# ai-dynamo/dynamo

Measured on AMD Instinct MI355X. Metric: output tok/s (node), Llama-3-70B serving, ISL8192/OSL1024, conc 16/GPU, higher is better.
Workload: dtype bf16; 1 GPU; model=llama-3-70b, global_batch=16, seq_len=8192, osl=1024, parallelism=agg1, kv_cache_dtype=auto

## Files before the change

### dynamo_amd/csrc/attention_decode.hip

```cpp
#include "attention_decode_impl.h"
#include <torch/extension.h>
#include <ATen/hip/HIPContext.h>

using namespace decode_attn;

int64_t paged_decode_num_chunks(int64_t max_ctx) {
  const int chunk = decode_chunk_tokens((int)max_ctx);
  return std::max<int64_t>(1, (max_ctx + chunk - 1) / chunk);
}

int64_t decode_chunk_tokens_py(int64_t max_ctx) {
  return decode_chunk_tokens((int)max_ctx);
}

void paged_attention_decode(torch::Tensor out, torch::Tensor q,
                            torch::Tensor kcache, torch::Tensor vcache,
                            torch::Tensor page_table, torch::Tensor ctx_lens,
                            torch::Tensor partial, torch::Tensor ml,
                            double scale, int64_t chunk_tokens,
                            bool v_transposed,
                            c10::optional<torch::Tensor> chunk_cnt) {
  TORCH_CHECK(q.is_cuda() && q.dtype() == torch::kBFloat16);
  TORCH_CHECK(page_table.dtype() == torch::kInt32 && ctx_lens.dtype() == torch::kInt32);
  const bool fp8 = kcache.dtype() == torch::kFloat8_e4m3fn;
  TORCH_CHECK(fp8 || kcache.dtype() == torch::kBFloat16,
              "kv cache must be bf16 or float8_e4m3fn");
  const int B = q.size(0);
  const int Hq = q.size(1);
  const int hd = q.size(2);
  const int Hkv = kcache.size(1);
  const int ps = kcache.size(2);
  const int G = Hq / Hkv;
  const int max_pages = page_table.size(1);
  const int C = ml.size(2);
  TORCH_CHECK(hd == 128, "only head_dim=128 supported natively");
  TORCH_CHECK((ps & (ps - 1)) == 0, "page_size must be a power of 2");
  int log2_ps = 0; while ((1 << log2_ps) < ps) log2_ps++;
  if (B == 0) return;
  const int chunk = (int)chunk_tokens;
  TORCH_CHECK(chunk >= 128 && chunk % 128 == 0, "bad chunk_tokens ", chunk);
  auto stream = at::cuda::getCurrentHIPStream();
  dim3 grid(B, Hkv, C);

  if (v_transposed) {
    TORCH_CHECK(vcache.size(2) == hd && vcache.size(3) == ps,
                "v_transposed expects vcache [P, Hkv, hd, ps]");
    TORCH_CHECK(ps % 32 == 0 && hd == 128 && G >= 2 && G <= 16,
                "v_transposed decode needs page_size%32==0, head_dim==128, "
                "2<=G<=16 (got G=", G, ")");
    const int lds = mfma_swapped_lds_bytes(G, hd, 72);
    static const bool use_fused_merge = [] {
      const char* e = getenv("DYNAMO_FUSED_MERGE");
      return e != nullptr && e[0] == '1';
    }();
    int32_t* cnt = nullptr;
    if (use_fused_merge && C > 1 && chunk_cnt.has_value() &&
        chunk_cnt->numel() >= (int64_t)B * Hkv)
      cnt = chunk_cnt->data_ptr<int32_t>();
    auto launch_vt = [&](auto* kern) {
      if (lds > 65536)
        (void)hipFuncSetAttribute(reinterpret_cast<const void*>(kern),
                                  hipFuncAttributeMaxDynamicSharedMemorySize,
                                  lds);
      kern<<<grid, kBlock, lds, stream>>>(
          partial.data_ptr<float>(), ml.data_ptr<float>(),
          (short*)out.data_ptr(), (const short*)q.data_ptr(),
          (const short*)kcache.data_ptr(), (const short*)vcache.data_ptr(),
          page_table.data_ptr<int32_t>(), ctx_lens.data_ptr<int32_t>(),
          (float)scale, chunk, G, B, Hkv, C, max_pages, log2_ps, hd, cnt);
    };
    static const int vt3v = [] {
      const char* e = getenv("DYNAMO_VT3_VARIANT");
      return e ? atoi(e) : 0;
    }();
    if (fp8)
      launch_vt(&paged_decode_mfma_swapped<1, 1, 0, 1, 72, 0, 4>);
    else if (vt3v == 1)
      launch_vt(&paged_decode_mfma_swapped<1, 1, 0, 0, 72, 0, 3, 0, 2>);
    else if (vt3v == 2)
      launch_vt(&paged_decode_mfma_swapped<1, 1, 0, 0, 72, 0, 2>);
    else if (vt3v == 5 && ps == 64)
      launch_vt(&paged_decode_mfma_swapped<1, 1, 0, 0, 72, 0, 5>);
    else
      launch_vt(&paged_decode_mfma_swapped<1, 1, 0, 0, 72, 0, 4>);
    HIP_CHECK_KERNEL();
    if (C > 1 && cnt == nullptr) {
      dim3 grid2(B, Hq);
      paged_decode_phase2<<<grid2, 128, 0, stream>>>(
          (short*)out.data_ptr(), partial.data_ptr<float>(),
          ml.data_ptr<float>(), ctx_lens.data_ptr<int32_t>(), chunk, Hq, C,
          hd);
      HIP_CHECK_KERNEL();
    }
    return;
  }

#define LAUNCH_G(GG, DP, HS, DEPTH)                                           \
  paged_decode_phase1<GG, DP, HS, DEPTH>                                      \
      <<<grid, kBlock, phase1_lds_bytes(GG, HS, hd), stream>>>(               \
      partial.data_ptr<float>(), ml.data_ptr<float>(), (short*)out.data_ptr(),\
      (const short*)q.data_ptr(), (const short*)kcache.data_ptr(),            \
      (const short*)vcache.data_ptr(), page_table.data_ptr<int32_t>(),        \
      ctx_lens.data_ptr<int32_t>(), (float)scale, chunk, B, Hkv, C,            \
      max_pages, log2_ps, hd)
  static const bool use_mfma = [] {
    const char* e = getenv("DYNAMO_DECODE_MFMA");
    return e == nullptr || e[0] != '0';
  }();
  static const bool use_swapped = [] {
    const char* e = getenv("DYNAMO_DECODE_SWAPPED");
    return e == nullptr || e[0] != '0';
  }();
#define LAUNCH_MFMA(GG)                                                       \
  do {                                                                        \
    if (use_swapped) {                                                        \
      if (mfma_swapped_lds_bytes(GG, hd, 72) > 65536)                             \
        (void)hipFuncSetAttribute(                                            \
            reinterpret_cast<const void*>(                                    \
                &paged_decode_mfma_swapped<1, 1, 0, 0, 72, 1>),                         \
            hipFuncAttributeMaxDynamicSharedMemorySize,                       \
            mfma_swapped_lds_bytes(GG, hd, 72));                                  \
      paged_decode_mfma_swapped<1, 1, 0, 0, 72, 1>                                      \
          <<<grid, kBlock, mfma_swapped_lds_bytes(GG, hd, 72), stream>>>(         \
          partial.data_ptr<float>(), ml.data_ptr<float>(),                    \
          (short*)out.data_ptr(), (const short*)q.data_ptr(),                 \
          (const short*)kcache.data_ptr(),                                    \
          (const short*)vcache.data_ptr(), page_table.data_ptr<int32_t>(),    \
          ctx_lens.data_ptr<int32_t>(), (float)scale, chunk, GG, B, Hkv, C,    \
          max_pages, log2_ps, hd, nullptr);                                   \
      break;                                                                  \
    }                                                                         \
    if (mfma_lds_bytes(GG, hd) > 65536)                                       \
      (void)hipFuncSetAttribute(                                              \
          reinterpret_cast<const void*>(&paged_decode_mfma<1, 1>),            \
          hipFuncAttributeMaxDynamicSharedMemorySize,                         \
          mfma_lds_bytes(GG, hd));                                            \
    paged_decode_mfma<1, 1><<<grid, kBlock, mfma_lds_bytes(GG, hd), stream>>>(\
      partial.data_ptr<float>(), ml.data_ptr<float>(), (short*)out.data_ptr(),\
      (const short*)q.data_ptr(), (const short*)kcache.data_ptr(),            \
      (const short*)vcache.data_ptr(), page_table.data_ptr<int32_t>(),        \
      ctx_lens.data_ptr<int32_t>(), (float)scale, chunk, GG, B, Hkv, C,        \
      max_pages, log2_ps, hd);                                                \
  } while (0)
  const bool mfma_ok = use_mfma && ps % 32 == 0 && hd == 128;
  if (fp8) {
    TORCH_CHECK(ps % 32 == 0 && hd == 128 && G <= 16,
                "fp8 KV cache needs page_size%32==0, head_dim==128, G<=16");
    if (mfma_swapped_lds_bytes(G, hd, 72) > 65536)
      (void)hipFuncSetAttribute(
          reinterpret_cast<const void*>(&paged_decode_mfma_swapped<1, 1, 0, 1, 72, 1>),
          hipFuncAttributeMaxDynamicSharedMemorySize,
          mfma_swapped_lds_bytes(G, hd, 72));
    paged_decode_mfma_swapped<1, 1, 0, 1, 72, 1>
        <<<grid, kBlock, mfma_swapped_lds_bytes(G, hd, 72), stream>>>(
        partial.data_ptr<float>(), ml.data_ptr<float>(),
        (short*)out.data_ptr(), (const short*)q.data_ptr(),
        (const short*)kcache.data_ptr(), (const short*)vcache.data_ptr(),
        page_table.data_ptr<int32_t>(), ctx_lens.data_ptr<int32_t>(),
        (float)scale, chunk, G, B, Hkv, C, max_pages, log2_ps, hd, nullptr);
// ... 43 lines not shown
```

### dynamo_amd/csrc/attention_decode_impl.h

```cpp
#pragma once
#include "common.h"
#include <cstdlib>

namespace decode_attn {

constexpr int kBlock = 256;

inline int decode_chunk_tokens(int max_ctx) {
#ifndef __HIP_DEVICE_COMPILE__
  if (const char* e = getenv("DYNAMO_DECODE_CHUNK")) {
    const int v = atoi(e);
    if (v >= 128 && v % 128 == 0) return v;
  }
#endif
  if (max_ctx >= 8192) return 2048;
  if (max_ctx >= 2048) return 1024;
  return 512;
}
#ifndef DECODE_KCHUNK
#define DECODE_KCHUNK 512
#endif
constexpr int kChunk = DECODE_KCHUNK;
constexpr float kNegInf = -1e30f;

// ... 389 lines not shown
      *(short*)((char*)p_lds + row * 64 + (((16 + lr) * 2) ^ x)) = f32_to_bf16(pB[r]);
    }
    __builtin_amdgcn_wave_barrier();
    asm volatile("s_waitcnt lgkmcnt(0)" ::: "memory");
    __builtin_amdgcn_sched_barrier(0);

    if (active) {
    short8 pa_s;
    {
      const int row = lr;
      const int x = (row & 3) << 4;
      pa_s = *reinterpret_cast<const short8*>(
          (char*)p_lds + row * 64 + ((lg * 16) ^ x));
    }
    bf16x8_t pa = *reinterpret_cast<bf16x8_t*>(&pa_s);
    if constexpr (PRIO) __builtin_amdgcn_s_setprio(1);
#pragma unroll
    for (int db = 0; db < 8; db++) {
      short8 vb_s = *reinterpret_cast<const short8*>(
          (const char*)v_lds + (db * 16 + lr) * 80 + lg * 16);
      bf16x8_t vbf = *reinterpret_cast<bf16x8_t*>(&vb_s);
      acc[db] = __builtin_amdgcn_mfma_f32_16x16x32_bf16(pa, vbf, acc[db],
                                                        0, 0, 0);
    }
    if constexpr (PRIO) __builtin_amdgcn_s_setprio(0);
    }
    __builtin_amdgcn_wave_barrier();
  }

  __syncthreads();
  float* my = merge + wid * G * (hd + 2);
#pragma unroll
  for (int r = 0; r < 4; r++) {
    const int row = lg * 4 + r;
    if (row < G) {
#pragma unroll
      for (int db = 0; db < 8; db++)
        my[row * (hd + 2) + db * 16 + lr] = acc[db][r];
      if (lr == 0) {
        my[row * (hd + 2) + hd] = m[r];
        my[row * (hd + 2) + hd + 1] = l[r];
      }
    }
  }
  __syncthreads();

  for (int i = threadIdx.x; i < G * hd; i += kBlock) {
    const int g = i / hd;
    const int d = i % hd;
    float mw[4], lw[4];
    float mstar = kNegInf;
#pragma unroll
    for (int w = 0; w < 4; w++) {
      mw[w] = merge[w * G * (hd + 2) + g * (hd + 2) + hd];
      lw[w] = merge[w * G * (hd + 2) + g * (hd + 2) + hd + 1];
      mstar = fmaxf(mstar, mw[w]);
    }
    float lsum = 0.f, asum = 0.f;
#pragma unroll
    for (int w = 0; w < 4; w++) {
      const float corr = (lw[w] > 0.f) ? __expf(mw[w] - mstar) : 0.f;
      lsum += lw[w] * corr;
      asum += merge[w * G * (hd + 2) + g * (hd + 2) + d] * corr;
    }
    const int qh = h * G + g;
    if (C == 1) {
      out[((int64_t)b * Hq + qh) * hd + d] =
          f32_to_bf16(lsum > 0.f ? asum / lsum : 0.f);
    } else {
      partial[(((int64_t)b * Hq + qh) * C + c) * hd + d] = asum;
      if (d == 0) {
        float* mlp = ml + (((int64_t)b * Hq + qh) * C + c) * 2;
        mlp[0] = mstar; mlp[1] = lsum;
      }
    }
  }
}

inline int mfma_lds_bytes(int G, int hd) {
  return 4 * G * (hd + 2) * 4 + G * hd * 2 + 4 * 5120 * 2 + 4 * 512 * 2;
}

template <int DEFER = 1, int PRIO = 1, int KPF = 0, int FP8 = 0,
          int VS = 80, int XK2 = 0, int VT = 0, int LG2 = 0, int MINW = 1>
__global__ __launch_bounds__(kBlock, MINW) void paged_decode_mfma_swapped(
    float* __restrict__ partial, float* __restrict__ ml,
    short* __restrict__ out, const short* __restrict__ q,
    const short* __restrict__ kcache, const short* __restrict__ vcache,
    const int32_t* __restrict__ page_table, const int32_t* __restrict__ ctx_lens,
    float scale, int chunk, int G, int B, int Hkv, int C, int max_pages,
    int log2_ps, int hd, int32_t* __restrict__ chunk_cnt) {
  typedef __attribute__((ext_vector_type(8))) __bf16 bf16x8_t;
  typedef __attribute__((ext_vector_type(2))) unsigned int uint2_t;
  const int kSlab = chunk / 4;
  const int b = blockIdx.x;
  const int h = blockIdx.y;
  const int c = blockIdx.z;
  const int Hq = Hkv * G;
  const int ctx = ctx_lens[b];
  const int chunk_start = c * chunk;
  const int lane = threadIdx.x & 63;
  const int wid = threadIdx.x >> 6;
  const int lr = lane & 15;
  const int lg = lane >> 4;
  const int ps = 1 << log2_ps;

  extern __shared__ float lds[];
  float* merge = lds;
  short* q_lds_s = reinterpret_cast<short*>(merge + 4 * G * (hd + 2));
  short* v_lds = q_lds_s + G * hd + wid * (hd * VS / 2);

  auto fused_merge = [&]() {
    __threadfence();
    __shared__ int lastflag;
    if (threadIdx.x == 0) {
      const int prev = atomicAdd(&chunk_cnt[b * Hkv + h], 1);
      lastflag = (prev == (int)gridDim.z - 1) ? 1 : 0;
    }
    __syncthreads();
    if (!lastflag) return;
    __threadfence();
    if (threadIdx.x == 0) chunk_cnt[b * Hkv + h] = 0;
    const int nc = min(C, (ctx + chunk - 1) / chunk);
    for (int i = threadIdx.x; i < G * hd; i += kBlock) {
      const int g = i / hd;
      const int d = i % hd;
      const int qh = h * G + g;
      const float* mlp = ml + (((int64_t)b * Hq + qh) * C) * 2;
      float mstar = kNegInf;
      for (int cc = 0; cc < nc; cc++) mstar = fmaxf(mstar, mlp[2 * cc]);
      float asum = 0.f, lsum2 = 0.f;
      for (int cc = 0; cc < nc; cc++) {
        const float lc = mlp[2 * cc + 1];
        if (lc <= 0.f) continue;
        const float corr = __expf(mlp[2 * cc] - mstar);
        asum += partial[(((int64_t)b * Hq + qh) * C + cc) * hd + d] * corr;
        lsum2 += lc * corr;
      }
      out[((int64_t)b * Hq + qh) * hd + d] =
          f32_to_bf16(lsum2 > 0.f ? asum / lsum2 : 0.f);
    }
  };

  if (chunk_start >= ctx) {
    if (C > 1) {
      for (int i = threadIdx.x; i < G; i += kBlock) {
        const int qh = h * G + i;
        float* mlp = ml + (((int64_t)b * Hq + qh) * C + c) * 2;
        mlp[0] = kNegInf; mlp[1] = 0.f;
      }
      if (chunk_cnt != nullptr) fused_merge();
    }
    return;
  }

  for (int i = threadIdx.x; i < G * hd; i += kBlock) {
    const int g = i / hd;
    q_lds_s[i] = q[((int64_t)b * Hq + h * G + g) * hd + i % hd];
  }
  __syncthreads();

  bf16x8_t q_frag[4];
#pragma unroll
  for (int kc = 0; kc < 4; kc++) {
    short8 v{};
    if (lr < G)
      v = *reinterpret_cast<const short8*>(q_lds_s + lr * hd + kc * 32 + lg * 8);
    q_frag[kc] = *reinterpret_cast<bf16x8_t*>(&v);
  }

  float m_run = kNegInf, l_run = 0.f;
  f32x4 acc[8];
#pragma unroll
  for (int d = 0; d < 8; d++) acc[d] = f32x4{0.f, 0.f, 0.f, 0.f};

  const int slab_start = chunk_start + wid * kSlab;
  const int slab_end = min(slab_start + kSlab, ctx);
  const int32_t* pt = page_table + (int64_t)b * max_pages;

  typedef __attribute__((ext_vector_type(4))) short short4v;
  auto ld8 = [&](const short* base, int64_t elem_off) -> short8 {
    if constexpr (FP8) {
      const unsigned char* b =
          reinterpret_cast<const unsigned char*>(base) + elem_off;
      uchar8 raw = *reinterpret_cast<const uchar8*>(b);
      bf16x8 cv = fp8x8_to_bf16x8(raw);
      return *reinterpret_cast<short8*>(&cv);
    } else {
      return *reinterpret_cast<const short8*>(base + elem_off);
    }
  };
  auto load_k = [&](int t0_, short8 (&kf)[8]) {
    if (t0_ >= slab_end) return;
    const int64_t pb = (((int64_t)pt[t0_ >> log2_ps] * Hkv + h) * ps) * hd;
    const int tA = t0_ + lr, tB = t0_ + 16 + lr;
    const int64_t oA = pb + (int64_t)(tA & (ps - 1)) * hd;
    const int64_t oB = pb + (int64_t)(tB & (ps - 1)) * hd;
    const bool vA = tA < slab_end, vB = tB < slab_end;
#pragma unroll
    for (int kc = 0; kc < 4; kc++) {
      kf[kc] = vA ? ld8(kcache, oA + kc * 32 + lg * 8) : short8{};
      kf[4 + kc] = vB ? ld8(kcache, oB + kc * 32 + lg * 8) : short8{};
    }
  };
  auto load_v = [&](int t0_, short8 (&vf)[8]) {
    if (t0_ >= slab_end) return;
    const int64_t pb = (((int64_t)pt[t0_ >> log2_ps] * Hkv + h) * ps) * hd;
#pragma unroll
    for (int u = 0; u < 2; u++) {
      const int unit = lane + u * 64;
      const int d8 = unit & 15;
      const int tg = unit >> 4;
#pragma unroll
      for (int j = 0; j < 4; j++) {
        const int t = t0_ + tg * 4 + j;
        vf[u * 4 + j] = (t < slab_end)
            ? ld8(vcache, pb + (int64_t)(t & (ps - 1)) * hd + d8 * 8)
            : short8{};
      }
    }
  };
  auto load_vt = [&](int t0_, short8 (&vf)[8]) {
    const int64_t pb = (((int64_t)pt[t0_ >> log2_ps] * Hkv + h) * ps) * hd;
    const int tin = t0_ & (ps - 1);
#pragma unroll
    for (int da = 0; da < 8; da++) {
      const int vrow = da * 16 + lr;
      vf[da] = ld8(vcache, pb + (int64_t)vrow * ps + tin + lg * 8);
    }
    const int rem = slab_end - t0_;
    if (rem < 32) {
#pragma unroll
      for (int da = 0; da < 8; da++)
#pragma unroll
        for (int j = 0; j < 8; j++)
          if (lg * 8 + j >= rem) vf[da][j] = 0;
    }
  };
  auto store_v = [&](const short8 (&vf)[8]) {
#pragma unroll
    for (int u = 0; u < 2; u++) {
      const int unit = lane + u * 64;
      const int d8 = unit & 15;
      const int tg = unit >> 4;
#pragma unroll
      for (int i = 0; i < 8; i++) {
        const int d = d8 * 8 + i;
        short4v pk = {vf[u * 4 + 0][i], vf[u * 4 + 1][i],
                      vf[u * 4 + 2][i], vf[u * 4 + 3][i]};
        const int toff = XK2 ? ((tg * 8) ^ (((d >> 4) & 1) << 5)) : (tg * 8);
        *reinterpret_cast<short4v*>((char*)v_lds + d * VS + toff) = pk;
      }
    }
  };

  short8 kfr[2][8], vfr[2][8];
  if constexpr (KPF) {
    load_k(slab_start, kfr[0]);
    load_v(slab_start, vfr[0]);
  }

  const float scale2 = scale * 1.44269504f;
  auto tile_vt = [&](int t0, const short8 (&kf)[8], const short8 (&vf)[8]) {
    f32x4 sA{0.f, 0.f, 0.f, 0.f}, sB{0.f, 0.f, 0.f, 0.f};
    if constexpr (PRIO) __builtin_amdgcn_s_setprio(1);
#pragma unroll
    for (int kc = 0; kc < 4; kc++) {
      short8 ka = kf[kc];
      sA = __builtin_amdgcn_mfma_f32_16x16x32_bf16(
          *reinterpret_cast<bf16x8_t*>(&ka), q_frag[kc], sA, 0, 0, 0);
    }
    if (t0 + 16 < slab_end) {
// ... 613 lines not shown
```

### dynamo_amd/csrc/bindings.cpp

```cpp
#include <torch/extension.h>
#include <pybind11/pybind11.h>

namespace py = pybind11;

void rmsnorm(torch::Tensor out, torch::Tensor input, torch::Tensor weight,
             double eps, bool allow_fast);
void fused_add_rmsnorm(torch::Tensor input, torch::Tensor residual,
                       torch::Tensor weight, double eps, bool allow_fast);
void rope_append_qkv(torch::Tensor q_out, torch::Tensor kcache,
                     torch::Tensor vcache, torch::Tensor qkv,
                     c10::optional<torch::Tensor> bias,
                     torch::Tensor positions, torch::Tensor slot_mapping,
                     torch::Tensor cos_sin_cache, bool v_transposed,
                     bool allow_fast);
void rope_inplace(torch::Tensor q, torch::Tensor k, torch::Tensor positions,
                  torch::Tensor cos_sin_cache, int64_t num_q_heads,
                  int64_t num_k_heads, int64_t head_dim);
void silu_mul(torch::Tensor out, torch::Tensor gate_up);
void gelu(torch::Tensor out, torch::Tensor input);
void kv_cache_append(torch::Tensor kcache, torch::Tensor vcache, torch::Tensor k,
                     torch::Tensor v, torch::Tensor slot_mapping,
                     bool v_transposed);
void gather_pages(torch::Tensor staging, torch::Tensor cache, torch::Tensor page_ids);
void scatter_pages(torch::Tensor staging, torch::Tensor cache, torch::Tensor page_ids);
void copy_pages(torch::Tensor dst_cache, torch::Tensor src_cache, torch::Tensor pairs);
int64_t paged_decode_num_chunks(int64_t max_ctx);
int64_t decode_chunk_tokens_py(int64_t max_ctx);
void paged_attention_decode(torch::Tensor out, torch::Tensor q, torch::Tensor kcache,
                            torch::Tensor vcache, torch::Tensor page_table,
                            torch::Tensor ctx_lens, torch::Tensor partial,
                            torch::Tensor ml, double scale,
                            int64_t chunk_tokens, bool v_transposed,
                            c10::optional<torch::Tensor> chunk_cnt);
void attention_prefill_paged(torch::Tensor out, torch::Tensor q,
                             torch::Tensor kcache, torch::Tensor vcache,
                             torch::Tensor page_table, torch::Tensor tile_seq,
                             torch::Tensor tile_q0, torch::Tensor seq_q_start,
                             torch::Tensor seq_q_len, torch::Tensor seq_ctx_len,
                             double scale, bool v_transposed);
void greedy_sample(torch::Tensor out, torch::Tensor logits, bool allow_fast);
void topkp_sample(torch::Tensor out, torch::Tensor logits,
                  torch::Tensor inv_temp, torch::Tensor top_k,
                  torch::Tensor top_p, int64_t seed,
                  c10::optional<torch::Tensor> row_seeds);
void gumbel_sample(torch::Tensor out, torch::Tensor logits, torch::Tensor inv_temp,
                   int64_t seed, c10::optional<torch::Tensor> row_seeds,
                   bool allow_fast);
void moe_grouped_gemm(torch::Tensor y, torch::Tensor x, torch::Tensor w,
                      torch::Tensor tiles);
void moe_grouped_gemm_seg(torch::Tensor y, torch::Tensor x, torch::Tensor w,
                          torch::Tensor seg_start, int64_t max_tokens);
void topk_gating(torch::Tensor topw, torch::Tensor topi, torch::Tensor logits);
torch::Tensor ipc_alloc(int64_t nbytes, int64_t device);
py::bytes ipc_export(torch::Tensor t);
torch::Tensor ipc_open(py::bytes handle_bytes, int64_t nbytes, int64_t device);
void enable_peer_access(int64_t device, int64_t peer);
torch::Tensor mfma_probe(torch::Tensor A, torch::Tensor B);
torch::Tensor tr16_probe();
torch::Tensor vstage_probe();
torch::Tensor pv_probe(int64_t hot);

PYBIND11_MODULE(TORCH_EXTENSION_NAME, m) {
  m.doc() = "dynamo_amd native MI355X (gfx950) kernels";
  m.def("rmsnorm", &rmsnorm, py::arg("out"), py::arg("input"),
        py::arg("weight"), py::arg("eps"), py::arg("allow_fast") = true);
  m.def("fused_add_rmsnorm", &fused_add_rmsnorm, py::arg("input"),
        py::arg("residual"), py::arg("weight"), py::arg("eps"),
        py::arg("allow_fast") = true);
  m.def("rope_inplace", &rope_inplace);
  m.def("rope_append_qkv", &rope_append_qkv,
        py::arg("q_out"), py::arg("kcache"), py::arg("vcache"),
        py::arg("qkv"), py::arg("bias"), py::arg("positions"),
        py::arg("slot_mapping"), py::arg("cos_sin"),
        py::arg("v_transposed") = false, py::arg("allow_fast") = true);
  m.def("silu_mul", &silu_mul);
  m.def("gelu", &gelu);
  m.def("kv_cache_append", &kv_cache_append, py::arg("kcache"),
        py::arg("vcache"), py::arg("k"), py::arg("v"),
        py::arg("slot_mapping"), py::arg("v_transposed") = false);
  m.def("gather_pages", &gather_pages);
  m.def("scatter_pages", &scatter_pages);
  m.def("copy_pages", &copy_pages);
  m.def("paged_decode_num_chunks", &paged_decode_num_chunks);
  m.def("decode_chunk_tokens", &decode_chunk_tokens_py);
  m.def("paged_attention_decode", &paged_attention_decode,
        py::arg("out"), py::arg("q"), py::arg("kcache"), py::arg("vcache"),
        py::arg("page_table"), py::arg("ctx_lens"), py::arg("partial"),
        py::arg("ml"), py::arg("scale"), py::arg("chunk_tokens"),
        py::arg("v_transposed") = false,
        py::arg("chunk_cnt") = py::none());
  m.def("attention_prefill_paged", &attention_prefill_paged,
        py::arg("out"), py::arg("q"), py::arg("kcache"), py::arg("vcache"),
        py::arg("page_table"), py::arg("tile_seq"), py::arg("tile_q0"),
        py::arg("seq_q_start"), py::arg("seq_q_len"), py::arg("seq_ctx_len"),
        py::arg("scale"), py::arg("v_transposed") = false);
  m.def("greedy_sample", &greedy_sample, py::arg("out"), py::arg("logits"),
        py::arg("allow_fast") = true);
  m.def("gumbel_sample", &gumbel_sample, py::arg("out"), py::arg("logits"),
        py::arg("inv_temp"), py::arg("seed"),
        py::arg("row_seeds") = py::none(), py::arg("allow_fast") = true);
  m.def("topkp_sample", &topkp_sample, py::arg("out"), py::arg("logits"),
        py::arg("inv_temp"), py::arg("top_k"), py::arg("top_p"),
        py::arg("seed"), py::arg("row_seeds") = py::none());
  m.def("moe_grouped_gemm", &moe_grouped_gemm);
  m.def("moe_grouped_gemm_seg", &moe_grouped_gemm_seg);
  m.def("topk_gating", &topk_gating);
  m.def("ipc_alloc", &ipc_alloc);
  m.def("ipc_export", &ipc_export);
  m.def("ipc_open", &ipc_open);
  m.def("enable_peer_access", &enable_peer_access);
  m.def("mfma_probe", &mfma_probe);
  m.def("tr16_probe", &tr16_probe);
  m.def("vstage_probe", &vstage_probe);
  m.def("pv_probe", &pv_probe);
}
```

### dynamo_amd/envs.py

```python
from __future__ import annotations

import os

ENV_VARS = {
    "DYN_DISCOVERY_BACKEND": "discovery backend spec: memory | file:/path",
    "DYN_NAMESPACE": "default namespace for components",
    "DYN_LOG": "log level (INFO, DEBUG, ...)",
    "DYN_LOGGING_JSONL": "1 = structured JSONL logs",
    "DYN_REQUEST_TRACE_FILE": "JSONL request-trace sink path",
    "DYN_HTTP_PORT": "frontend HTTP port",
    "DYN_ROUTER_MODE": "kv | round_robin | random | least_loaded | p2c",
    "DYN_ROUTER_TEMPERATURE": "softmax temperature for kv routing",
    "DYN_KV_BLOCK_SIZE": "KV page size in tokens",
    "DYN_KV_GPU_MEM_FRACTION": "fraction of free HBM for the KV pool",
    "DYN_HOST_CACHE_PAGES": "KVBM G2 pinned-host tier size (pages)",
    "DYN_TUNABLEOP": "0 disables the pre-tuned hipBLASLt table",
    "DYN_WORKER_TYPE": "aggregated | prefill | decode",
    "DYN_BYPASS_TOKEN_THRESHOLD":
        "conditional disagg: net-new prefill tokens below this bypass the "
        "prefill pool (reference conditional_disagg.rs:15; default 2048)",
    "DYNAMO_DECODE_CHUNK": "decode attention context-chunk tokens override",
    "DYNAMO_DECODE_MFMA": "0 = force the VALU decode path (token-major only)",
    "DYNAMO_DECODE_SWAPPED": "0 = A-operand MFMA decode (token-major only)",
    "DYNAMO_VT3_VARIANT":
        "d-major decode variant select: 0=VT4 (default), 1=VT3, 2=VT2, "
        "5=VT5 (recorded-negative V-LDS variant)",
    "DYNAMO_FUSED_MERGE":
        "1 = fused decode chunk merge (recorded-negative; threadfence cost)",
    "DYNAMO_MOE_BMM": "0 = grouped-kernel MoE decode instead of padded bmm",
    "DYNAMO_MOE_MFMA": "0 = VALU grouped MoE GEMM",
    "DYNAMO_MOE_GRAPHS": "0 = exclude MoE layers from hipGraph capture",
    "DYNAMO_ROCTX": "1 = roctx range annotations for rocprofv3 traces",
}


def get(name: str, default=None, cast=str):
    v = os.environ.get(name)
    if v is None:
        return default
    try:
        if cast is bool:
            return v not in ("0", "false", "False", "")
        return cast(v)
    except (TypeError, ValueError):
        return default


def discovery(default="memory"):
    return get("DYN_DISCOVERY_BACKEND", default)


def namespace(default="dynamo"):
    return get("DYN_NAMESPACE", default)
```

### dynamo_amd/models/layers.py

```python
from __future__ import annotations

from dataclasses import dataclass, field
from typing import List, Optional

import torch
import torch.nn.functional as F

from dynamo_amd import ops


@dataclass
class AttnMetadata:
    slot_mapping: torch.Tensor
    positions: torch.Tensor
    num_decode: int = 0
    decode_page_table: Optional[torch.Tensor] = None
    decode_ctx_lens: Optional[torch.Tensor] = None
    decode_scratch: Optional["ops.DecodeScratch"] = None
    num_prefill_tokens: int = 0
    prefill_page_table: Optional[torch.Tensor] = None
    seq_q_start: Optional[torch.Tensor] = None
    seq_q_len: Optional[torch.Tensor] = None
    seq_ctx_len: Optional[torch.Tensor] = None
    prefill_tiles: Optional[tuple] = None
    logits_rows: Optional[torch.Tensor] = None
    embeds_rows: Optional[torch.Tensor] = None
    inputs_embeds: Optional[torch.Tensor] = None
    v_transposed: bool = False


def linear(x: torch.Tensor, w: torch.Tensor) -> torch.Tensor:
    return F.linear(x, w)


def linear_lora(x: torch.Tensor, w: torch.Tensor, lora, key: str) -> torch.Tensor:
    y = F.linear(x, w)
    if lora is not None and key in lora:
        A, B, scale = lora[key]
        y = y + F.linear(F.linear(x, A), B) * scale
    return y


class TPContext:

    def __init__(self, tp_size: int = 1, tp_rank: int = 0, group=None):
        self.size = tp_size
        self.rank = tp_rank
        self.group = group

    def all_reduce(self, x: torch.Tensor) -> torch.Tensor:
        if self.size > 1:
            torch.distributed.all_reduce(x, group=self.group)
        return x


_DEFAULT_TP = TPContext()


def _alloc(shape, device, dtype):
    from dynamo_amd.gms import current_allocator
    pool = current_allocator()
    if pool is not None:
        return pool.allocate(shape, dtype), pool.needs_init
    return torch.empty(shape, device=device, dtype=dtype), True


def init_weight(shape, device, dtype, std=0.02, generator=None):
    from dynamo_amd.gms import current_allocator
    pooled = current_allocator() is not None
    w, needs = _alloc(shape, device, dtype)
    if needs:
        with torch.no_grad():
            if pooled:
                tmp = torch.empty(shape, device=device, dtype=dtype)
                tmp.normal_(0.0, std, generator=generator)
                w.copy_(tmp)
            else:
                w.normal_(0.0, std, generator=generator)
    return w


def init_const(shape, device, dtype, val=1.0):
    w, needs = _alloc(shape, device, dtype)
    if needs:
        with torch.no_grad():
            w.fill_(val)
    return w


def init_sharded(shape, device, dtype, tp: "TPContext", dim: int, std=0.02):
    if tp.size == 1:
        return init_weight(shape, device, dtype, std)
    n = shape[dim] // tp.size
    shard_shape = list(shape)
    shard_shape[dim] = n
    shard, needs = _alloc(tuple(shard_shape), device, dtype)
    if needs:
        full = torch.empty(shape, device=device, dtype=dtype)
        with torch.no_grad():
            full.normal_(0.0, std)
        shard.copy_(full.narrow(dim, tp.rank * n, n))
        del full
    return shard


class Attention(torch.nn.Module):

    def __init__(self, cfg, layer_idx: int, tp: TPContext, device, dtype):
        super().__init__()
        self.layer_idx = layer_idx
        self.tp = tp
        self.hq = cfg.num_q_heads // tp.size
        self.hkv = max(1, cfg.num_kv_heads // tp.size)
        self.hd = cfg.head_dim
        self.scale = self.hd ** -0.5
        D = cfg.hidden_size
        qkv_rows = (self.hq + 2 * self.hkv) * self.hd
        kv_idx = (tp.rank if tp.size <= cfg.num_kv_heads
                  else (tp.rank * cfg.num_kv_heads) // tp.size)
# ... 84 lines not shown
```

### dynamo_amd/ops/__init__.py

```python
from __future__ import annotations

import torch

from . import torch_ref
from .torch_ref import make_cos_sin_cache

_hip_mod = None
_hip_err: Exception | None = None


def hip():
    global _hip_mod, _hip_err
    if _hip_mod is None:
        try:
            from dynamo_amd import _hip as m
            _hip_mod = m
        except Exception as e:
            _hip_err = e
            raise RuntimeError(
                "dynamo_amd._hip native extension is not available on a GPU "
                "device path. Build it with `python setup.py build_ext "
                f"--inplace` (PYTORCH_ROCM_ARCH=gfx950). Original error: {e}"
            ) from e
    return _hip_mod


def hip_available() -> bool:
    try:
        hip()
        return True
    except RuntimeError:
        return False


def rmsnorm(x: torch.Tensor, weight: torch.Tensor, eps: float,
            allow_fast: bool = True) -> torch.Tensor:
    if x.is_cuda:
        out = torch.empty_like(x)
        hip().rmsnorm(out, x.contiguous(), weight, eps, allow_fast)
        return out
    return torch_ref.rmsnorm(x, weight, eps)


def fused_add_rmsnorm(x, residual, weight, eps, allow_fast=True):
    if x.is_cuda:
        hip().fused_add_rmsnorm(x, residual, weight, eps, allow_fast)
        return x
    return torch_ref.fused_add_rmsnorm(x, residual, weight, eps)


def rope_inplace(q, k, positions, cos_sin, num_q_heads, num_k_heads, head_dim):
    if q.is_cuda:
        hip().rope_inplace(q, k, positions, cos_sin, num_q_heads, num_k_heads,
                           head_dim)
        return q, k
    return torch_ref.rope(q, k, positions, cos_sin, num_q_heads, num_k_heads,
                          head_dim)


def silu_mul(gate_up: torch.Tensor) -> torch.Tensor:
    if gate_up.is_cuda:
        d = gate_up.shape[-1] // 2
        out = torch.empty(gate_up.shape[:-1] + (d,), dtype=gate_up.dtype,
                          device=gate_up.device)
        hip().silu_mul(out, gate_up.contiguous())
        return out
    return torch_ref.silu_mul(gate_up)


def gelu(x: torch.Tensor) -> torch.Tensor:
    if x.is_cuda:
        out = torch.empty_like(x)
        hip().gelu(out, x.contiguous())
        return out
    return torch_ref.gelu(x)


def kv_cache_append(kcache, vcache, k, v, slot_mapping,
                    v_transposed=False):
    if kcache.is_cuda:
        hip().kv_cache_append(kcache, vcache, k.contiguous(), v.contiguous(),
                              slot_mapping, v_transposed)
    else:
        torch_ref.kv_cache_append(kcache, vcache, k, v, slot_mapping,
                                  v_transposed)


def rope_append_qkv(qkv, bias, positions, slot_mapping, cos_sin,
                    kcache, vcache, num_q_heads, num_kv_heads, head_dim,
                    v_transposed=False, allow_fast=True):
    T = qkv.shape[0]
    if qkv.is_cuda:
        q_out = torch.empty(T, num_q_heads * head_dim, dtype=qkv.dtype,
                            device=qkv.device)
        hip().rope_append_qkv(q_out, kcache, vcache, qkv, bias, positions,
                              slot_mapping, cos_sin, v_transposed, allow_fast)
        return q_out
    if bias is not None:
        qkv = qkv + bias
    q, k, v = qkv.split([num_q_heads * head_dim, num_kv_heads * head_dim,
                         num_kv_heads * head_dim], dim=-1)
    q = q.contiguous()
    k = k.contiguous()
    q, k = torch_ref.rope(q, k, positions, cos_sin, num_q_heads,
                          num_kv_heads, head_dim)
    torch_ref.kv_cache_append(kcache, vcache, k.view(T, num_kv_heads, head_dim),
                              v.view(T, num_kv_heads, head_dim), slot_mapping,
                              v_transposed)
    return q


class DecodeScratch:

    def __init__(self, max_batch: int, num_q_heads: int, head_dim: int,
                 max_ctx: int, device):
        self.chunks = int(hip().paged_decode_num_chunks(max_ctx))
        self.chunk_tokens = int(hip().decode_chunk_tokens(max_ctx))
        self.partial = torch.empty(max_batch, num_q_heads, self.chunks, head_dim,
                                   dtype=torch.float32, device=device)
        self.ml = torch.empty(max_batch, num_q_heads, self.chunks, 2,
                              dtype=torch.float32, device=device)
        self.chunk_cnt = torch.zeros(max_batch * 128, dtype=torch.int32,
                                     device=device)

    def view(self, batch: int):
        return self.partial[:batch], self.ml[:batch]


def paged_attention_decode(q, kcache, vcache, page_table, ctx_lens, scale,
                           scratch: "DecodeScratch | None" = None, out=None,
                           v_transposed=False):
    if q.is_cuda:
        if out is None:
            out = torch.empty_like(q)
        assert scratch is not None, "GPU decode needs a DecodeScratch"
        partial, ml = scratch.view(q.shape[0])
        hip().paged_attention_decode(out, q, kcache, vcache, page_table,
                                     ctx_lens, partial, ml, scale,
                                     scratch.chunk_tokens, v_transposed,
                                     scratch.chunk_cnt)
        return out
    r = torch_ref.paged_attention_decode(q, kcache, vcache, page_table,
                                         ctx_lens, scale,
                                         v_transposed=v_transposed)
    if out is not None:
        out.copy_(r)
        return out
    return r


def prefill_tile_rows(num_q_heads: int, num_kv_heads: int) -> int:
    if num_q_heads % num_kv_heads == 0:
        g = num_q_heads // num_kv_heads
        if g in (2, 4, 8):
            return (8 // g) * 32
    return 64


def build_prefill_tiles(seq_q_lens, device, rows: int = 64):
    tile_seq, tile_q0 = [], []
    for s, ql in enumerate(seq_q_lens):
        for q0 in range(0, int(ql), rows):
            tile_seq.append(s)
            tile_q0.append(q0)
    return (torch.tensor(tile_seq, dtype=torch.int32, device=device),
            torch.tensor(tile_q0, dtype=torch.int32, device=device))


def attention_prefill_paged(q, kcache, vcache, page_table, seq_q_start,
                            seq_q_len, seq_ctx_len, scale, tiles=None,
                            v_transposed=False):
    if q.is_cuda:
        out = torch.empty_like(q)
        if tiles is None:
            rows = prefill_tile_rows(q.shape[1], kcache.shape[1])
            tiles = build_prefill_tiles(seq_q_len.tolist(), q.device, rows)
        tile_seq, tile_q0 = tiles
        hip().attention_prefill_paged(out, q, kcache, vcache, page_table,
                                      tile_seq, tile_q0, seq_q_start,
                                      seq_q_len, seq_ctx_len, scale,
                                      v_transposed)
        return out
    return torch_ref.attention_prefill_paged(q, kcache, vcache, page_table,
                                             seq_q_start, seq_q_len,
                                             seq_ctx_len, scale,
                                             v_transposed=v_transposed)


def greedy_sample(logits: torch.Tensor, allow_fast: bool = True) -> torch.Tensor:
    if logits.is_cuda:
        out = torch.empty(logits.shape[0], dtype=torch.int32,
                          device=logits.device)
        hip().greedy_sample(out, logits.float().contiguous(), allow_fast)
        return out
    return torch_ref.greedy_sample(logits)


def _splitmix64(x: torch.Tensor) -> torch.Tensor:
    def lsr(v, k):
        return (v >> k) & ((1 << (64 - k)) - 1)
    x = x + 0x9e3779b97f4a7c15
    x = (x ^ lsr(x, 30)) * -0x40a7b892e31b1a47
    x = (x ^ lsr(x, 27)) * -0x6b2fb644ecceee15
    return x ^ lsr(x, 31)


def gumbel_sample(logits: torch.Tensor, inv_temp: torch.Tensor,
                  seed: int, row_seeds: torch.Tensor = None,
                  allow_fast: bool = True) -> torch.Tensor:
    if logits.is_cuda:
        out = torch.empty(logits.shape[0], dtype=torch.int32,
                          device=logits.device)
        hip().gumbel_sample(out, logits.float().contiguous(), inv_temp, seed,
                            row_seeds, allow_fast)
        return out
    B, V = logits.shape
    if row_seeds is None:
        rs = (torch.tensor(seed, dtype=torch.int64)
              ^ (torch.arange(B, dtype=torch.int64) << 32))
    else:
        rs = row_seeds.to(torch.int64).cpu()
    v = torch.arange(V, dtype=torch.int64).unsqueeze(0)
    h = _splitmix64(rs.unsqueeze(1) ^ v)
# ... 78 lines not shown
```

### setup.py

```python
import os
import sys

os.environ.setdefault("PYTORCH_ROCM_ARCH", "gfx950")

from setuptools import setup
from torch.utils.cpp_extension import BuildExtension, CppExtension, CUDAExtension

ROOT = os.path.dirname(os.path.abspath(__file__))
CSRC = os.path.join(ROOT, "dynamo_amd", "csrc")

hip_sources = [
    os.path.join(CSRC, f)
    for f in (
        "bindings.cpp",
        "norm.hip",
        "rope.hip",
        "activation.hip",
        "cache.hip",
        "attention_decode.hip",
        "attention_prefill.hip",
        "sampling.hip",
        "moe.hip",
        "ipc.hip",
        "probe.hip",
    )
]

ext_modules = [
    CUDAExtension(
        name="dynamo_amd._hip",
        sources=hip_sources,
        extra_compile_args={
            "cxx": ["-O3", "-std=c++17"],
            "nvcc": ["-O3", "-std=c++17", "--offload-arch=gfx950"],
        },
    ),
    CppExtension(
        name="dynamo_amd._core",
        sources=[os.path.join(CSRC, "core", "core.cpp")],
        extra_compile_args=["-O3", "-std=c++17"],
    ),
]

setup(
    name="dynamo_amd",
    version="0.1.0",
    packages=["dynamo_amd"],
    ext_modules=ext_modules,
    cmdclass={"build_ext": BuildExtension.with_options(use_ninja=True)},
)
```

Before: 429.9 tok/s.

## Add skinny-M MFMA GEMM for the decode MLP projection and an opt-in non-temporal KV load path

Adds an in-tree skinny-M bf16 GEMM kernel for M<=16 that splits K across waves with an LDS reduction, plus a coalesced variant that uses ds_bpermute to reshuffle weight fragments. It is routed through a new ops.linear for the (57344, 8192) shape, which is the fused gate/up projection in Llama-70B, and is meant to beat hipBLASLt on decode-time, weight-bandwidth-bound GEMMs. It also adds an opt-in non-temporal load template for K/V reads in decode attention, which is off by default. The risk is that the hand-written kernel underuses bandwidth compared with the tuned library on this shape.

```diff
diff --git a/dynamo_amd/csrc/attention_decode.hip b/dynamo_amd/csrc/attention_decode.hip
--- a/dynamo_amd/csrc/attention_decode.hip
+++ b/dynamo_amd/csrc/attention_decode.hip
@@ -3,6 +3,8 @@
 #include <ATen/hip/HIPContext.h>
 
 using namespace decode_attn;
+
+static constexpr bool kDecodeNtDefault = false;
 
 int64_t paged_decode_num_chunks(int64_t max_ctx) {
   const int chunk = decode_chunk_tokens((int)max_ctx);
@@ -19,7 +21,8 @@
                             torch::Tensor partial, torch::Tensor ml,
                             double scale, int64_t chunk_tokens,
                             bool v_transposed,
-                            c10::optional<torch::Tensor> chunk_cnt) {
+                            c10::optional<torch::Tensor> chunk_cnt,
+                            int64_t nt_policy) {
   TORCH_CHECK(q.is_cuda() && q.dtype() == torch::kBFloat16);
   TORCH_CHECK(page_table.dtype() == torch::kInt32 && ctx_lens.dtype() == torch::kInt32);
   const bool fp8 = kcache.dtype() == torch::kFloat8_e4m3fn;
@@ -73,8 +76,17 @@
       const char* e = getenv("DYNAMO_VT3_VARIANT");
       return e ? atoi(e) : 0;
     }();
-    if (fp8)
+    static const bool nt_env = [] {
+      const char* e = getenv("DYNAMO_DECODE_NT");
+      return e == nullptr ? kDecodeNtDefault : e[0] != '0';
+    }();
+    const bool use_nt = nt_policy < 0 ? nt_env : nt_policy != 0;
+    if (fp8 && use_nt)
+      launch_vt(&paged_decode_mfma_swapped<1, 1, 0, 1, 72, 0, 4, 0, 1, 1>);
+    else if (fp8)
       launch_vt(&paged_decode_mfma_swapped<1, 1, 0, 1, 72, 0, 4>);
+    else if (vt3v == 0 && use_nt)
+      launch_vt(&paged_decode_mfma_swapped<1, 1, 0, 0, 72, 0, 4, 0, 1, 1>);
     else if (vt3v == 1)
       launch_vt(&paged_decode_mfma_swapped<1, 1, 0, 0, 72, 0, 3, 0, 2>);
     else if (vt3v == 2)
diff --git a/dynamo_amd/csrc/attention_decode_impl.h b/dynamo_amd/csrc/attention_decode_impl.h
--- a/dynamo_amd/csrc/attention_decode_impl.h
+++ b/dynamo_amd/csrc/attention_decode_impl.h
@@ -495,7 +495,8 @@
 }
 
 template <int DEFER = 1, int PRIO = 1, int KPF = 0, int FP8 = 0,
-          int VS = 80, int XK2 = 0, int VT = 0, int LG2 = 0, int MINW = 1>
+          int VS = 80, int XK2 = 0, int VT = 0, int LG2 = 0, int MINW = 1,
+          int NTKV = 0>
 __global__ __launch_bounds__(kBlock, MINW) void paged_decode_mfma_swapped(
     float* __restrict__ partial, float* __restrict__ ml,
     short* __restrict__ out, const short* __restrict__ q,
@@ -596,11 +597,19 @@
     if constexpr (FP8) {
       const unsigned char* b =
           reinterpret_cast<const unsigned char*>(base) + elem_off;
-      uchar8 raw = *reinterpret_cast<const uchar8*>(b);
+      uchar8 raw;
+      if constexpr (NTKV)
+        raw = __builtin_nontemporal_load(reinterpret_cast<const uchar8*>(b));
+      else
+        raw = *reinterpret_cast<const uchar8*>(b);
       bf16x8 cv = fp8x8_to_bf16x8(raw);
       return *reinterpret_cast<short8*>(&cv);
     } else {
-      return *reinterpret_cast<const short8*>(base + elem_off);
+      if constexpr (NTKV)
+        return __builtin_nontemporal_load(
+            reinterpret_cast<const short8*>(base + elem_off));
+      else
+        return *reinterpret_cast<const short8*>(base + elem_off);
     }
   };
   auto load_k = [&](int t0_, short8 (&kf)[8]) {
diff --git a/dynamo_amd/csrc/bindings.cpp b/dynamo_amd/csrc/bindings.cpp
--- a/dynamo_amd/csrc/bindings.cpp
+++ b/dynamo_amd/csrc/bindings.cpp
@@ -31,7 +31,8 @@
                             torch::Tensor ctx_lens, torch::Tensor partial,
                             torch::Tensor ml, double scale,
                             int64_t chunk_tokens, bool v_transposed,
-                            c10::optional<torch::Tensor> chunk_cnt);
+                            c10::optional<torch::Tensor> chunk_cnt,
+                            int64_t nt_policy);
 void attention_prefill_paged(torch::Tensor out, torch::Tensor q,
                              torch::Tensor kcache, torch::Tensor vcache,
                              torch::Tensor page_table, torch::Tensor tile_seq,
@@ -46,6 +47,9 @@
 void gumbel_sample(torch::Tensor out, torch::Tensor logits, torch::Tensor inv_temp,
                    int64_t seed, c10::optional<torch::Tensor> row_seeds,
                    bool allow_fast);
+void skinny_gemm(torch::Tensor y, torch::Tensor x, torch::Tensor w,
+                 int64_t wpb, int64_t u, int64_t nt, bool nontemporal,
+                 bool coalesced);
 void moe_grouped_gemm(torch::Tensor y, torch::Tensor x, torch::Tensor w,
                       torch::Tensor tiles);
 void moe_grouped_gemm_seg(torch::Tensor y, torch::Tensor x, torch::Tensor w,
@@ -88,7 +92,7 @@
         py::arg("page_table"), py::arg("ctx_lens"), py::arg("partial"),
         py::arg("ml"), py::arg("scale"), py::arg("chunk_tokens"),
         py::arg("v_transposed") = false,
-        py::arg("chunk_cnt") = py::none());
+        py::arg("chunk_cnt") = py::none(), py::arg("nt_policy") = -1);
   m.def("attention_prefill_paged", &attention_prefill_paged,
         py::arg("out"), py::arg("q"), py::arg("kcache"), py::arg("vcache"),
         py::arg("page_table"), py::arg("tile_seq"), py::arg("tile_q0"),
@@ -102,6 +106,9 @@
   m.def("topkp_sample", &topkp_sample, py::arg("out"), py::arg("logits"),
         py::arg("inv_temp"), py::arg("top_k"), py::arg("top_p"),
         py::arg("seed"), py::arg("row_seeds") = py::none());
+  m.def("skinny_gemm", &skinny_gemm, py::arg("y"), py::arg("x"), py::arg("w"),
+        py::arg("wpb") = 4, py::arg("u") = 4, py::arg("nt") = 2,
+        py::arg("nontemporal") = false, py::arg("coalesced") = false);
   m.def("moe_grouped_gemm", &moe_grouped_gemm);
   m.def("moe_grouped_gemm_seg", &moe_grouped_gemm_seg);
   m.def("topk_gating", &topk_gating);
diff --git a/dynamo_amd/csrc/skinny_gemm.hip b/dynamo_amd/csrc/skinny_gemm.hip
--- /dev/null
+++ b/dynamo_amd/csrc/skinny_gemm.hip
@@ -0,0 +1,64 @@
+#include "skinny_gemm_impl.h"
+#include <torch/extension.h>
+#include <ATen/hip/HIPContext.h>
+
+void skinny_gemm(torch::Tensor y, torch::Tensor x, torch::Tensor w,
+                 int64_t wpb, int64_t u, int64_t nt, bool nontemporal,
+                 bool coalesced) {
+  TORCH_CHECK(x.is_cuda() && w.is_cuda() && y.is_cuda(),
+              "skinny_gemm: tensors must be on the GPU");
+  TORCH_CHECK(x.dtype() == torch::kBFloat16 && w.dtype() == torch::kBFloat16 &&
+                  y.dtype() == torch::kBFloat16,
+              "skinny_gemm: bf16 only");
+  TORCH_CHECK(x.dim() == 2 && w.dim() == 2 && y.dim() == 2,
+              "skinny_gemm: x [M,K], w [N,K], y [M,N]");
+  TORCH_CHECK(x.is_contiguous() && w.is_contiguous() && y.is_contiguous(),
+              "skinny_gemm: x, w and y must be contiguous");
+  const int64_t M = x.size(0), K = x.size(1), N = w.size(0);
+  TORCH_CHECK(w.size(1) == K && y.size(0) == M && y.size(1) == N,
+              "skinny_gemm: shape mismatch");
+  TORCH_CHECK(M >= 1 && M <= 16, "skinny_gemm: needs 1 <= M <= 16, got ", M);
+  TORCH_CHECK(N >= 16 && N % 16 == 0, "skinny_gemm: needs N % 16 == 0, got ", N);
+  TORCH_CHECK(N < (1 << 27), "skinny_gemm: N too large");
+  TORCH_CHECK(wpb > 0 && u > 0 && nt > 0, "skinny_gemm: bad configuration");
+  const int64_t kstep = wpb * (coalesced ? 64 : 32) * u;
+  TORCH_CHECK(K >= 2048 && K < (1 << 30) && K % kstep == 0,
+              "skinny_gemm: needs K >= 2048 and K % ", kstep, " == 0, got ", K);
+  auto stream = at::cuda::getCurrentHIPStream();
+  const short* xp = (const short*)x.data_ptr();
+  const short* wp = (const short*)w.data_ptr();
+  short* yp = (short*)y.data_ptr();
+  const int grid = (int)((N + nt * 16 - 1) / (nt * 16));
+
+  bool launched = false;
+#define SKINNY_CASE(WPB, U, NT)                                              \
+  if (!launched && wpb == WPB && u == U && nt == NT) {                       \
+    if (nontemporal)                                                         \
+      skinny::skinny_gemm_kernel<WPB, U, NT, 1>                              \
+          <<<grid, WPB * 64, 0, stream>>>(xp, wp, yp, (int)M, (int)N, (int)K); \
+    else                                                                     \
+      skinny::skinny_gemm_kernel<WPB, U, NT, 0>                              \
+          <<<grid, WPB * 64, 0, stream>>>(xp, wp, yp, (int)M, (int)N, (int)K); \
+    launched = true;                                                         \
+  }
+#define SKINNY_COAL_CASE(WPB, U2, NT)                                        \
+  if (!launched && wpb == WPB && u == U2 && nt == NT) {                      \
+    if (nontemporal)                                                         \
+      skinny::skinny_gemm_coal_kernel<WPB, U2, NT, 1>                        \
+          <<<grid, WPB * 64, 0, stream>>>(xp, wp, yp, (int)M, (int)N, (int)K); \
+    else                                                                     \
+      skinny::skinny_gemm_coal_kernel<WPB, U2, NT, 0>                        \
+          <<<grid, WPB * 64, 0, stream>>>(xp, wp, yp, (int)M, (int)N, (int)K); \
+    launched = true;                                                         \
+  }
+  if (coalesced) {
+    SKINNY_GEMM_COAL_CONFIGS(SKINNY_COAL_CASE)
+  } else {
+    SKINNY_GEMM_CONFIGS(SKINNY_CASE)
+  }
+#undef SKINNY_COAL_CASE
+#undef SKINNY_CASE
+  TORCH_CHECK(launched, "skinny_gemm: no kernel for (WPB, U, NT) = (", wpb,
+              ", ", u, ", ", nt, ")");
+  HIP_CHECK_KERNEL();
+}
diff --git a/dynamo_amd/csrc/skinny_gemm_impl.h b/dynamo_amd/csrc/skinny_gemm_impl.h
--- /dev/null
+++ b/dynamo_amd/csrc/skinny_gemm_impl.h
@@ -0,0 +1,228 @@
+#pragma once
+
+#include "common.h"
+
+namespace skinny {
+
+template <int NTL>
+DEVINL bf16x8 ldw(const short* p) {
+  if constexpr (NTL)
+    return __builtin_nontemporal_load(reinterpret_cast<const bf16x8*>(p));
+  else
+    return *reinterpret_cast<const bf16x8*>(p);
+}
+
+template <int WPB, int U, int NT, int NTL>
+__global__ __launch_bounds__(WPB * 64) void skinny_gemm_kernel(
+    const short* __restrict__ x,
+    const short* __restrict__ w,
+    short* __restrict__ y,
+    int M, int N, int K) {
+  const int lane = threadIdx.x & 63;
+  const int wid = threadIdx.x >> 6;
+  const int lr = lane & 15;
+  const int lg = lane >> 4;
+  const int n0 = (blockIdx.x * NT) * 16;
+  if (n0 >= N) return;
+
+  const int kw = K / WPB;
+  const int k0 = wid * kw;
+  const int steps = kw / 32;
+
+  const int ar = lr < M ? lr : 0;
+  const short* xp = x + (size_t)ar * K + k0 + lg * 8;
+  const short* wp[NT];
+#pragma unroll
+  for (int t = 0; t < NT; t++) {
+    const int col = n0 + t * 16 + lr;
+    wp[t] = w + (size_t)(col < N ? col : N - 1) * K + k0 + lg * 8;
+  }
+
+  f32x4 acc[NT];
+#pragma unroll
+  for (int t = 0; t < NT; t++) acc[t] = f32x4{0.f, 0.f, 0.f, 0.f};
+
+  bf16x8 abuf[U];
+  bf16x8 bbuf[NT][U];
+#pragma unroll
+  for (int u = 0; u < U; u++) {
+    abuf[u] = *reinterpret_cast<const bf16x8*>(xp + u * 32);
+#pragma unroll
+    for (int t = 0; t < NT; t++) bbuf[t][u] = ldw<NTL>(wp[t] + u * 32);
+  }
+
+  for (int s = U; s < steps; s += U) {
+#pragma unroll
+    for (int u = 0; u < U; u++) {
+      bf16x8 a = abuf[u];
+      abuf[u] = *reinterpret_cast<const bf16x8*>(xp + (s + u) * 32);
+#pragma unroll
+      for (int t = 0; t < NT; t++) {
+        bf16x8 b = bbuf[t][u];
+        bbuf[t][u] = ldw<NTL>(wp[t] + (s + u) * 32);
+        acc[t] = __builtin_amdgcn_mfma_f32_16x16x32_bf16(a, b, acc[t], 0, 0, 0);
+      }
+    }
+  }
+#pragma unroll
+  for (int u = 0; u < U; u++)
+#pragma unroll
+    for (int t = 0; t < NT; t++)
+      acc[t] = __builtin_amdgcn_mfma_f32_16x16x32_bf16(abuf[u], bbuf[t][u],
+                                                       acc[t], 0, 0, 0);
+
+  __shared__ f32x4 red[WPB > 1 ? (WPB - 1) * NT * 64 : 1];
+  if (WPB > 1) {
+    if (wid > 0) {
+#pragma unroll
+      for (int t = 0; t < NT; t++)
+        red[((wid - 1) * NT + t) * 64 + lane] = acc[t];
+    }
+    __syncthreads();
+    if (wid > 0) return;
+#pragma unroll
+    for (int t = 0; t < NT; t++)
+#pragma unroll
+      for (int r = 0; r < WPB - 1; r++) {
+        f32x4 o = red[(r * NT + t) * 64 + lane];
+        acc[t].x += o.x; acc[t].y += o.y; acc[t].z += o.z; acc[t].w += o.w;
+      }
+  }
+#pragma unroll
+  for (int t = 0; t < NT; t++) {
+    const int col = n0 + t * 16 + lr;
+    if (col >= N) continue;
+#pragma unroll
+    for (int i = 0; i < 4; i++) {
+      const int row = lg * 4 + i;
+      if (row < M)
+        y[(size_t)row * N + col] = f32_to_bf16(acc[t][i]);
+    }
+  }
+}
+
+template <int WPB, int U2, int NT, int NTL>
+__global__ __launch_bounds__(WPB * 64) void skinny_gemm_coal_kernel(
+    const short* __restrict__ x, const short* __restrict__ w,
+    short* __restrict__ y, int M, int N, int K) {
+  typedef __attribute__((ext_vector_type(4))) int int4v;
+  const int lane = threadIdx.x & 63;
+  const int wid = threadIdx.x >> 6;
+  const int lr = lane & 15;
+  const int lg = lane >> 4;
+  const int n0 = (blockIdx.x * NT) * 16;
+  if (n0 >= N) return;
+
+  const int kw = K / WPB;
+  const int k0 = wid * kw;
+  const int dsteps = kw / 64;
+
+  const int ar = lr < M ? lr : 0;
+  const short* xp = x + (size_t)ar * K + k0 + lg * 8;
+  const short* wp[NT][2];
+#pragma unroll
+  for (int t = 0; t < NT; t++)
+#pragma unroll
+    for (int h = 0; h < 2; h++) {
+      const int col = n0 + t * 16 + h * 8 + (lane >> 3);
+      wp[t][h] = w + (size_t)(col < N ? col : N - 1) * K + k0 + (lane & 7) * 8;
+    }
+  const int src0 = (8 * (lr & 7) + lg) * 4;
+  const bool hi = lr >= 8;
+
+  f32x4 acc[NT];
+#pragma unroll
+  for (int t = 0; t < NT; t++) acc[t] = f32x4{0.f, 0.f, 0.f, 0.f};
+
+  bf16x8 abuf[U2][2];
+  bf16x8 rbuf[NT][U2][2];
+#pragma unroll
+  for (int u = 0; u < U2; u++) {
+    abuf[u][0] = *reinterpret_cast<const bf16x8*>(xp + u * 64);
+    abuf[u][1] = *reinterpret_cast<const bf16x8*>(xp + u * 64 + 32);
+#pragma unroll
+    for (int t = 0; t < NT; t++) {
+      rbuf[t][u][0] = ldw<NTL>(wp[t][0] + u * 64);
+      rbuf[t][u][1] = ldw<NTL>(wp[t][1] + u * 64);
+    }
+  }
+
+  auto consume = [&](const bf16x8 (&a)[2], const bf16x8& r0, const bf16x8& r1,
+                     f32x4& c) {
+    const int4v v0 = *reinterpret_cast<const int4v*>(&r0);
+    const int4v v1 = *reinterpret_cast<const int4v*>(&r1);
+#pragma unroll
+    for (int s = 0; s < 2; s++) {
+      int4v b;
+#pragma unroll
+      for (int j = 0; j < 4; j++) {
+        const int t0 = __builtin_amdgcn_ds_bpermute(src0 + s * 16, v0[j]);
+        const int t1 = __builtin_amdgcn_ds_bpermute(src0 + s * 16, v1[j]);
+        b[j] = hi ? t1 : t0;
+      }
+      c = __builtin_amdgcn_mfma_f32_16x16x32_bf16(
+          a[s], *reinterpret_cast<const bf16x8*>(&b), c, 0, 0, 0);
+    }
+  };
+
+  for (int d = U2; d < dsteps; d += U2) {
+#pragma unroll
+    for (int u = 0; u < U2; u++) {
+      bf16x8 a[2] = {abuf[u][0], abuf[u][1]};
+      abuf[u][0] = *reinterpret_cast<const bf16x8*>(xp + (d + u) * 64);
+      abuf[u][1] = *reinterpret_cast<const bf16x8*>(xp + (d + u) * 64 + 32);
+#pragma unroll
+      for (int t = 0; t < NT; t++) {
+        bf16x8 r0 = rbuf[t][u][0], r1 = rbuf[t][u][1];
+        rbuf[t][u][0] = ldw<NTL>(wp[t][0] + (d + u) * 64);
+        rbuf[t][u][1] = ldw<NTL>(wp[t][1] + (d + u) * 64);
+        consume(a, r0, r1, acc[t]);
+      }
+    }
+  }
+#pragma unroll
+  for (int u = 0; u < U2; u++)
+#pragma unroll
+    for (int t = 0; t < NT; t++)
+      consume(abuf[u], rbuf[t][u][0], rbuf[t][u][1], acc[t]);
+
+  __shared__ f32x4 red[WPB > 1 ? (WPB - 1) * NT * 64 : 1];
+  if (WPB > 1) {
+    if (wid > 0) {
+#pragma unroll
+      for (int t = 0; t < NT; t++)
+        red[((wid - 1) * NT + t) * 64 + lane] = acc[t];
+    }
+    __syncthreads();
+    if (wid > 0) return;
+#pragma unroll
+    for (int t = 0; t < NT; t++)
+#pragma unroll
+      for (int r = 0; r < WPB - 1; r++) {
+        f32x4 o = red[(r * NT + t) * 64 + lane];
+        acc[t].x += o.x; acc[t].y += o.y; acc[t].z += o.z; acc[t].w += o.w;
+      }
+  }
+#pragma unroll
+  for (int t = 0; t < NT; t++) {
+    const int col = n0 + t * 16 + lr;
+    if (col >= N) continue;
+#pragma unroll
+    for (int i = 0; i < 4; i++) {
+      const int row = lg * 4 + i;
+      if (row < M)
+        y[(size_t)row * N + col] = f32_to_bf16(acc[t][i]);
+    }
+  }
+}
+
+#define SKINNY_GEMM_COAL_CONFIGS(X)                                         \
+  X(8, 1, 2) X(8, 1, 4) X(8, 2, 2) X(4, 2, 2) X(8, 2, 4) X(2, 2, 8)          \
+  X(1, 4, 2) X(1, 2, 4) X(1, 4, 4) X(1, 8, 2) X(1, 2, 2) X(1, 1, 8) X(1, 2, 8)
+
+#define SKINNY_GEMM_CONFIGS(X)                                              \
+  X(4, 4, 2) X(4, 4, 4) X(4, 2, 4) X(2, 4, 4) X(2, 8, 4)                    \
+  X(1, 8, 4) X(1, 4, 8) X(2, 4, 8) X(4, 8, 2) X(2, 2, 8) X(4, 8, 4)          \
+  X(8, 4, 2) X(16, 4, 2) X(16, 2, 2) X(8, 4, 1) X(16, 4, 1) X(8, 2, 4)
+
+}
diff --git a/dynamo_amd/envs.py b/dynamo_amd/envs.py
--- a/dynamo_amd/envs.py
+++ b/dynamo_amd/envs.py
@@ -27,6 +27,12 @@
         "5=VT5 (recorded-negative V-LDS variant)",
     "DYNAMO_FUSED_MERGE":
         "1 = fused decode chunk merge (recorded-negative; threadfence cost)",
+    "DYNAMO_DECODE_NT":
+        "1 = non-temporal K/V loads in the d-major (VT4) decode attention "
+        "kernel (bit-identical outputs; recorded-negative, slower)",
+    "DYNAMO_SKINNY_GEMM":
+        "0 = every decode weight GEMM on hipBLASLt (default: the in-tree "
+        "skinny-M kernel on the shapes in ops.SKINNY_GEMM_SHAPES)",
     "DYNAMO_MOE_BMM": "0 = grouped-kernel MoE decode instead of padded bmm",
     "DYNAMO_MOE_MFMA": "0 = VALU grouped MoE GEMM",
     "DYNAMO_MOE_GRAPHS": "0 = exclude MoE layers from hipGraph capture",
diff --git a/dynamo_amd/models/layers.py b/dynamo_amd/models/layers.py
--- a/dynamo_amd/models/layers.py
+++ b/dynamo_amd/models/layers.py
@@ -30,11 +30,11 @@
 
 
 def linear(x: torch.Tensor, w: torch.Tensor) -> torch.Tensor:
-    return F.linear(x, w)
+    return ops.linear(x, w)
 
 
 def linear_lora(x: torch.Tensor, w: torch.Tensor, lora, key: str) -> torch.Tensor:
-    y = F.linear(x, w)
+    y = ops.linear(x, w)
     if lora is not None and key in lora:
         A, B, scale = lora[key]
         y = y + F.linear(F.linear(x, A), B) * scale
diff --git a/dynamo_amd/ops/__init__.py b/dynamo_amd/ops/__init__.py
--- a/dynamo_amd/ops/__init__.py
+++ b/dynamo_amd/ops/__init__.py
@@ -31,6 +31,51 @@
         return True
     except RuntimeError:
         return False
+
+
+SKINNY_GEMM_SHAPES: dict = {
+    (57344, 8192): (1, 2, 2, True, True),
+}
+
+_skinny_override: "bool | None" = None
+
+
+def set_skinny_gemm(on: "bool | None") -> None:
+    global _skinny_override
+    _skinny_override = on
+
+
+def skinny_gemm_enabled() -> bool:
+    if _skinny_override is not None:
+        return _skinny_override
+    from dynamo_amd import envs
+    return envs.get("DYNAMO_SKINNY_GEMM", True, bool)
+
+
+def skinny_gemm_config(x: torch.Tensor, w: torch.Tensor):
+    if not (x.is_cuda and x.dim() == 2 and w.dim() == 2
+            and x.dtype == torch.bfloat16 and w.dtype == torch.bfloat16):
+        return None
+    M, K = x.shape
+    N = w.shape[0]
+    cfg = SKINNY_GEMM_SHAPES.get((N, K))
+    if cfg is None or not 1 <= M <= 16 or w.shape[1] != K:
+        return None
+    kstep = cfg[0] * cfg[1] * (64 if len(cfg) > 4 and cfg[4] else 32)
+    if N % 16 or K < 2048 or K % kstep:
+        return None
+    if not (x.is_contiguous() and w.is_contiguous()):
+        return None
+    return cfg if skinny_gemm_enabled() else None
+
+
+def linear(x: torch.Tensor, w: torch.Tensor) -> torch.Tensor:
+    cfg = skinny_gemm_config(x, w)
+    if cfg is None:
+        return torch.nn.functional.linear(x, w)
+    y = torch.empty(x.shape[0], w.shape[0], dtype=x.dtype, device=x.device)
+    hip().skinny_gemm(y, x, w, *cfg)
+    return y
 
 
 def rmsnorm(x: torch.Tensor, weight: torch.Tensor, eps: float,
@@ -129,7 +174,7 @@
 
 def paged_attention_decode(q, kcache, vcache, page_table, ctx_lens, scale,
                            scratch: "DecodeScratch | None" = None, out=None,
-                           v_transposed=False):
+                           v_transposed=False, nt_policy: int = -1):
     if q.is_cuda:
         if out is None:
             out = torch.empty_like(q)
@@ -138,7 +183,7 @@
         hip().paged_attention_decode(out, q, kcache, vcache, page_table,
                                      ctx_lens, partial, ml, scale,
                                      scratch.chunk_tokens, v_transposed,
-                                     scratch.chunk_cnt)
+                                     scratch.chunk_cnt, nt_policy)
         return out
     r = torch_ref.paged_attention_decode(q, kcache, vcache, page_table,
                                          ctx_lens, scale,
diff --git a/setup.py b/setup.py
--- a/setup.py
+++ b/setup.py
@@ -19,6 +19,7 @@
         "cache.hip",
         "attention_decode.hip",
         "attention_prefill.hip",
+        "skinny_gemm.hip",
         "sampling.hip",
         "moe.hip",
         "ipc.hip",
```

Result: faster. 456.1 tok/s (median of 6 runs) (+6.1%).
